# AaltoML/SLAM-module

Measured on AMD Instinct MI355X. Metric: frames/sec ORB extract+match (720p), higher is better.
Workload: dtype u8; 1 GPU; C2+C3: ORB extract 1280x720, 8 levels x1.2, 2000 kpts/frame, FAST thr 20, batch 256 synthetic frames/GPU, + Hamming brute-force best2 + ratio 0.75 of each frame vs the previous (256 pairs, <=2000x2000); batch_per_gpu=256, corner_density=7-9 % of pixels (tools/synth.py defaults)

## Files before the change

include/mi355slam.h:

```cpp
#ifndef MI355SLAM_H
#define MI355SLAM_H

#include <stddef.h>
#include <stdint.h>

#ifdef __cplusplus
extern "C" {
#endif

#define MS_MAX_LEVELS 16
#define MS_ORB_PATCH_RADIUS 19
#define MS_HAMMING_THR_LOW 50
#define MS_HAMMING_THR_HIGH 100
#define MS_HAMMING_MAX 256

typedef enum {
    MS_OK = 0,
    MS_ERR_INVALID = -1,
    MS_ERR_NO_DEVICE = -2,
    MS_ERR_HIP = -3,
    MS_ERR_CAPACITY = -4,
    MS_ERR_NUMERIC = -5,
    MS_ERR_TOO_LATE = -6
} ms_status;
// ... 45 lines not shown
typedef struct {
    int32_t capacity;
    int32_t *count;
    float *x, *y;
    float *angle;
    int32_t *octave;
    uint32_t *desc;
    int32_t *track_id;
} ms_keypoints;

int ms_orb_create(ms_ctx *ctx, const ms_orb_config *cfg, ms_orb **out);
void ms_orb_destroy(ms_orb *orb);

int ms_orb_set_valid_mask(ms_orb *orb, const uint8_t *mask_host);

int ms_orb_extract(ms_orb *orb, const uint8_t *images, int images_on_device, int n_frames,
                   size_t frame_stride, size_t row_stride,
                   const float *track_xy, const int32_t *track_id, const int32_t *n_tracks);

int ms_orb_device_view(ms_orb *orb, ms_keypoints *view);
int ms_orb_download(ms_orb *orb, int frame, float *x, float *y, float *angle, int32_t *octave,
                    uint32_t *desc, int32_t *track_id, int32_t *n);
int ms_orb_capacity(const ms_orb *orb);

#define MS_KEYPOINT_RECORD_BYTES 76
int ms_keypoints_pack(ms_ctx *ctx, const ms_keypoints *view, int frame, int n, const double *bearing, uint8_t *records_host);
int ms_keypoints_unpack(const uint8_t *records, int n, float *x, float *y, float *angle, int32_t *octave, double *bearing, uint32_t *desc);

int ms_orb_set_describe_strip(ms_orb *orb, int r);

int ms_orb_set_resize_plan(ms_orb *orb, int px, int map);

int ms_orb_set_describe_order(ms_orb *orb, int mode);

#define MS_ORB_STAGES 6
int ms_orb_set_profiling(ms_orb *orb, int enable);
int ms_orb_stage_ms(ms_orb *orb, float *ms );
int ms_orb_stage_ms_back(ms_orb *orb, int calls_back, float *ms );
int ms_orb_level_size(const ms_orb *orb, int level, int32_t *w, int32_t *h);
int ms_orb_download_level(ms_orb *orb, int frame, int level, int blurred, uint8_t *dst_host);
int ms_orb_download_detections(ms_orb *orb, int frame, int level, int32_t *x, int32_t *y, int32_t *score, int32_t *n);
int ms_orb_last_candidate_counts(ms_orb *orb, int32_t *out );

int ms_hamming_set_path(ms_ctx *ctx, int path);

int ms_hamming_best2(ms_ctx *ctx, const uint32_t *q, int nq, const uint32_t *t, int nt, int n_pairs,
                     const int32_t *q_bucket, const int32_t *t_bucket, const uint8_t *t_valid,
                     int32_t *best_idx, uint16_t *best_dist, uint16_t *second_dist);

int ms_hamming_best2_sets(ms_ctx *ctx, const uint32_t *q_pool, int q_stride, const int32_t *q_count,
                          const uint32_t *t_pool, int t_stride, const int32_t *t_count,
                          const int32_t *pair_q, const int32_t *pair_t, int n_pairs,
                          int32_t *best_idx, uint16_t *best_dist, uint16_t *second_dist);

int ms_ratio_test(ms_ctx *ctx, const int32_t *best_idx, const uint16_t *best_dist, const uint16_t *second_dist,
                  int n, float lowe_ratio, int max_dist, int32_t *match);

int ms_hamming_candidates(ms_ctx *ctx, const uint32_t *q_desc, int nq, const uint32_t *t_desc,
                          const int32_t *cand_start, const int32_t *cand_idx, const uint8_t *t_skip, const int32_t *t_octave,
                          int32_t *best_idx, uint16_t *best_dist, uint16_t *second_dist, int32_t *best_octave, int32_t *second_octave,
                          int32_t *second_idx );

#define MS_MEDOID_MAX_OBS 256
int ms_descriptor_medoid(ms_ctx *ctx, const uint32_t *desc_pool, const int32_t *obs_start, const int32_t *obs_idx, int n_points,
                         int max_obs, int32_t *best_local, int32_t *best_pool);

// ... 608 lines not shown
```

slam-module_amd/csrc/orb.hip:

```cpp
#include "ms_internal.h"
#include "fast_tiles.h"
#include "describe_order.h"
#include "describe_strips.h"
#include "describe_lanes.h"
#include "describe_steer.h"
#include "describe_brief_index.h"
#include "resize_vpass.h"
#include "resize_plan.h"
#include "orb_geom.h"
#include <cfloat>
#include <cmath>
#include <cstring>

namespace {

using describe_lanes::kHalfPatch;

__device__ __forceinline__ int tile_level(const TileMap &tm, int levels, int t) {
    int l = 0;
#pragma unroll
    for (int k = 1; k < MS_MAX_LEVELS; ++k) l += t >= tm.base[k] ? 1 : 0;
    return l;
}

// ... 358 lines not shown
        for (int r = 0; r < kBlurRows + 6; ++r) {
            const uint8_t *row = img + (uint64_t)reflect101(y0 - 3 + r, h) * pitch;
            uint32_t d = reinterpret_cast<const U32u *>(row + xa)->v;
            if (wave_l) {
                const uint32_t f0 = reinterpret_cast<const U32u *>(row)->v, f1 = reinterpret_cast<const U32u *>(row + 4)->v;
                d = is_l ? __builtin_amdgcn_perm(f1, f0, 0x01020304u) : d;
            }
            if (wave_r) {
                const uint32_t e0 = reinterpret_cast<const U32u *>(row + (w - 8))->v, e1 = reinterpret_cast<const U32u *>(row + (w - 4))->v;
                d = is_r ? __builtin_amdgcn_perm(e1, e0, sel_r) : d;
            }
            e[r] = d & 0x00FF00FFu;
            o[r] = (d >> 8) & 0x00FF00FFu;
        }
    }
    uint8_t *dst = src.slab + (uint64_t)f * TL.slab_stride + G.blur_off;
#pragma unroll
    for (int j = 0; j < kBlurRows; ++j) {
        const uint32_t Ce = vsum7(e + j), Co = vsum7(o + j);
        const uint32_t Le = wave_from_prev(Ce), Lo = wave_from_prev(Co);
        const uint32_t Re = wave_from_next(Ce), Ro = wave_from_next(Co);
        uint32_t o0 = dot2(Lo, 18, 48, 32768u); o0 = dot2(Le, 0, 34, o0); o0 = dot2(Ce, 56, 34, o0); o0 = dot2(Co, 48, 18, o0);
        uint32_t o1 = dot2(Le, 0, 18, 32768u); o1 = dot2(Lo, 0, 34, o1); o1 = dot2(Ce, 48, 48, o1); o1 = dot2(Co, 56, 34, o1); o1 = dot2(Re, 18, 0, o1);
        uint32_t o2 = dot2(Lo, 0, 18, 32768u); o2 = dot2(Ce, 34, 56, o2); o2 = dot2(Co, 48, 48, o2); o2 = dot2(Re, 34, 0, o2); o2 = dot2(Ro, 18, 0, o2);
        uint32_t o3 = dot2(Ce, 18, 48, 32768u); o3 = dot2(Co, 34, 56, o3); o3 = dot2(Re, 48, 18, o3); o3 = dot2(Ro, 34, 0, o3);
        const int y = y0 + j;
        if (y < h && lane >= 1 && lane <= 62 && x < w)
            *reinterpret_cast<uint32_t *>(dst + (uint64_t)y * G.pitch + x) = (o0 >> 16) | ((o1 >> 16) << 8) | ((o2 >> 16) << 16) | ((o3 >> 16) << 24);
    }
}

constexpr int kFastWaves = 8, kFastThreads = 64 * kFastWaves;
constexpr int kFastSeg = 248, kFastRows = 4 * kFastWaves - 2, kFastPosRows = kFastRows + 2, kFastRowsPerWave = 4;
constexpr int kFastPruneMinBlocks = 2 * 4 * 256;
constexpr int kFastPositions = kFastPosRows * (kFastSeg + 2);

__device__ __forceinline__ uint32_t pk_sub(uint32_t a, uint32_t b) {
    return __builtin_bit_cast(uint32_t, (us2_t)(__builtin_bit_cast(us2_t, a) - __builtin_bit_cast(us2_t, b)));
}

__device__ __forceinline__ int mbcnt64(unsigned long long m) {
    return (int)__builtin_amdgcn_mbcnt_hi((uint32_t)(m >> 32), __builtin_amdgcn_mbcnt_lo((uint32_t)m, 0u));
}

__device__ __forceinline__ uint32_t pk_min(uint32_t a, uint32_t b) { return __builtin_bit_cast(uint32_t, __builtin_elementwise_min(__builtin_bit_cast(s2_t, a), __builtin_bit_cast(s2_t, b))); }
__device__ __forceinline__ uint32_t pk_max(uint32_t a, uint32_t b) { return __builtin_bit_cast(uint32_t, __builtin_elementwise_max(__builtin_bit_cast(s2_t, a), __builtin_bit_cast(s2_t, b))); }
__device__ __forceinline__ uint32_t compass_pass(uint32_t n, uint32_t s_, uint32_t e, uint32_t w, uint32_t c, uint32_t T2) {
    const uint32_t a = pk_max(n, s_), b = pk_min(n, s_), cx = pk_max(e, w), d = pk_min(e, w);
    return pk_sub(T2, pk_max(pk_sub(pk_min(a, cx), c), pk_sub(c, pk_max(b, d))));
}

__device__ __forceinline__ int arc_score(const s2_t P[8]) {
    s2_t pmn[8], smn[8];
    pmn[0] = P[0];
    smn[7] = P[7];
#pragma unroll
    for (int k = 1; k < 8; ++k) {
        pmn[k] = __builtin_elementwise_min(pmn[k - 1], P[k]);
        smn[7 - k] = __builtin_elementwise_min(smn[8 - k], P[7 - k]);
    }
    s2_t best = __builtin_elementwise_min(smn[0], pmn[0].yx);
#pragma unroll
    for (int k = 1; k < 8; ++k) best = __builtin_elementwise_max(best, __builtin_elementwise_min(smn[k], pmn[k].yx));
    return max((int)best.x, (int)best.y);
}

__device__ __forceinline__ s2_t pk_mad(uint32_t s, uint32_t r, uint32_t k) {
// ... 657 lines not shown
}

}

struct ms_orb {
    ms_ctx *ctx = nullptr;
    ms_orb_config cfg{};
    PyrGeom geom{};
    TileMap blur_tiles{};
    TileLevels tile_levels{};
    uint8_t *d_block = nullptr;
#define ORB_X_MEMBER(T, name, n) T *d_##name = nullptr;
#define ORB_XL_MEMBER(T, name, n) T *d_##name[MS_MAX_LEVELS] = {nullptr};
    ORB_BLOCK_CONSTANTS(ORB_X_MEMBER, ORB_XL_MEMBER)
    ORB_BLOCK_WORK(ORB_X_MEMBER)
#undef ORB_X_MEMBER
#undef ORB_XL_MEMBER
    size_t cand_count_bytes = 0, score_hist_bytes = 0;
    uint8_t *d_mask = nullptr;
    bool wide[MS_MAX_LEVELS] = {false};
    int resize_px = 0, resize_map = 0;
    int describe_order = describe_order::kDefaultMode;
    int describe_strip = 0;
    bool profiling = false;
    bool blur_valid = false;
    static constexpr int kProfRing = 128;
    hipEvent_t evr[kProfRing][MS_ORB_STAGES + 1] = {{nullptr}};
    hipEvent_t *ev = evr[0];
    long long prof_calls = 0;
    hipStream_t copy_stream = nullptr;
    hipEvent_t ev_copied[4] = {nullptr}, ev_free[4] = {nullptr}, ev_end = nullptr;
    int chunked_frames = 0;
    bool end_recorded = false;
    FrameSrc last_src{};
    int last_frames = 0;
    bool lvl0_in_slab = false;
    uint64_t lvl0_off = 0;
    int lvl0_pitch = 0;
};

#define MS_TRY(x) do { int rc__ = (x); if (rc__ != MS_OK) return rc__; } while (0)

__global__ __launch_bounds__(256) void k_pack_keypoints(const float *__restrict__ x, const float *__restrict__ y, const float *__restrict__ angle,
                                                       const int32_t *__restrict__ octave, const uint32_t *__restrict__ desc, const double *__restrict__ bearing,
                                                       uint64_t base, int n, uint32_t *__restrict__ out) {
    const int i = blockIdx.x * 256 + threadIdx.x;
    if (i >= n * 19) return;
    const int k = i / 19, w = i - 19 * k;
    const uint64_t s = base + (uint64_t)k;
    uint32_t v;
    if (w == 0) v = __float_as_uint(x[s]);
    else if (w == 1) v = __float_as_uint(y[s]);
    else if (w == 2) v = __float_as_uint(angle[s]);
    else if (w < 5) v = (uint32_t)octave[s];
    else if (w < 11) v = bearing ? reinterpret_cast<const uint32_t *>(bearing)[6 * (uint64_t)k + (w - 5)] : 0u;
    else v = desc[s * 8 + (w - 11)];
    out[i] = v;
}

static int orb_take_block(ms_orb *o, const OrbGeom &R, const OrbTables &C) {
    ms_ctx *c = o->ctx;
    const OrbBlock K = orb_block_layout(o->cfg, R, C);
    MS_HIP(c, hipMalloc(reinterpret_cast<void **>(&o->d_block), K.end));
#define ORB_X_BIND(T, name, n) o->d_##name = K.name.at(o->d_block);
#define ORB_XL_BIND(T, name, n) for (int l = 0; l < MS_MAX_LEVELS; ++l) o->d_##name[l] = K.name[l].count ? K.name[l].at(o->d_block) : nullptr;
    ORB_BLOCK_CONSTANTS(ORB_X_BIND, ORB_XL_BIND)
    ORB_BLOCK_WORK(ORB_X_BIND)
#undef ORB_X_BIND
#undef ORB_XL_BIND
    o->cand_count_bytes = K.cand_count.bytes(); o->score_hist_bytes = K.score_hist.bytes();
    std::vector<uint8_t> stage;
    orb_stage_constants(K, R, C, stage);
    MS_HIP(c, hipMemcpyAsync(o->d_block, stage.data(), K.const_end, hipMemcpyHostToDevice, c->stream));
    MS_HIP(c, hipMemsetAsync(o->d_block + K.const_end, 0, K.end - K.const_end, c->stream));
    MS_HIP(c, hipStreamSynchronize(c->stream));
    return MS_OK;
}

static int orb_create_streams(ms_orb *o) {
    ms_ctx *c = o->ctx;
    MS_HIP(c, hipEventCreateWithFlags(&o->ev_end, hipEventDisableTiming));
    if (o->cfg.max_batch < 32) return MS_OK;
    MS_HIP(c, hipStreamCreateWithFlags(&o->copy_stream, hipStreamNonBlocking));
    for (int i = 0; i < 4; ++i) {
        MS_HIP(c, hipEventCreateWithFlags(&o->ev_copied[i], hipEventDisableTiming));
        MS_HIP(c, hipEventCreateWithFlags(&o->ev_free[i], hipEventDisableTiming));
    }
    return MS_OK;
}

extern "C" {

int ms_orb_create(ms_ctx *ctx, const ms_orb_config *cfg, ms_orb **out) {
    if (!ctx || !cfg || !out) return MS_ERR_INVALID;
    *out = nullptr;
    OrbGeom R;
    char why[256];
    const int bad = orb_geometry(*cfg, R, why, sizeof(why));
    if (bad != MS_OK) return ms_fail(ctx, bad, "ms_orb_create: %s", why);
    OrbTables C;
    orb_tables(R.geom, C);
    MS_HIP(ctx, hipSetDevice(ctx->device));
    ms_orb *o = new ms_orb();
    o->ctx = ctx;
    o->cfg = *cfg;
    o->geom = R.geom; o->tile_levels = R.tile_levels; o->blur_tiles = R.blur_tiles;
    o->lvl0_off = R.lvl0_off; o->lvl0_pitch = R.lvl0_pitch;
    for (int l = 1; l < cfg->levels; ++l) o->wide[l] = C.level[l].wide;
    if (orb_take_block(o, R, C) != MS_OK) { ms_orb_destroy(o); return ms_fail(ctx, MS_ERR_HIP, "ms_orb_create: device allocation failed"); }
    if (orb_create_streams(o) != MS_OK) { ms_orb_destroy(o); return ms_fail(ctx, MS_ERR_HIP, "ms_orb_create: stream / event creation failed"); }
    *out = o;
    return MS_OK;
}

void ms_orb_destroy(ms_orb *o) {
    if (!o) return;
    (void)hipSetDevice(o->ctx->device);
    (void)hipStreamSynchronize(o->ctx->stream);
    if (o->d_block) (void)hipFree(o->d_block);
    if (o->d_mask) (void)hipFree(o->d_mask);
    for (auto &set : o->evr) for (int i = 0; i <= MS_ORB_STAGES; ++i) if (set[i]) (void)hipEventDestroy(set[i]);
    if (o->copy_stream) { (void)hipStreamSynchronize(o->copy_stream); (void)hipStreamDestroy(o->copy_stream); }
    for (int i = 0; i < 4; ++i) { if (o->ev_copied[i]) (void)hipEventDestroy(o->ev_copied[i]); if (o->ev_free[i]) (void)hipEventDestroy(o->ev_free[i]); }
    if (o->ev_end) (void)hipEventDestroy(o->ev_end);
    delete o;
}

int ms_orb_capacity(const ms_orb *o) { return o ? o->geom.capacity : MS_ERR_INVALID; }

int ms_orb_set_describe_strip(ms_orb *o, int r) {
    if (!o || r < 0 || r > describe_strips::kMaxStrip) return MS_ERR_INVALID;
    o->describe_strip = r;
    return MS_OK;
}

int ms_orb_set_resize_plan(ms_orb *o, int px, int map) {
    if (!o || (px != 0 && px != 4 && px != 8) || map < resize_plan::kMapAuto || map > resize_plan::kMapByFrame) return MS_ERR_INVALID;
    o->resize_px = px; o->resize_map = map;
    return MS_OK;
}

int ms_orb_set_describe_order(ms_orb *o, int mode) {
    if (!o || mode < 0 || (mode & ~describe_order::kModeMask)) return MS_ERR_INVALID;
    o->describe_order = mode;
    return MS_OK;
}

int ms_orb_set_profiling(ms_orb *o, int enable) {
    if (!o) return MS_ERR_INVALID;
    ms_ctx *c = o->ctx;
    if (enable && !o->evr[0][0])
        for (auto &set : o->evr) for (int i = 0; i <= MS_ORB_STAGES; ++i) MS_HIP(c, hipEventCreate(&set[i]));
    o->profiling = enable != 0;
    return MS_OK;
}

int ms_orb_stage_ms_back(ms_orb *o, int calls_back, float *ms) {
    if (!o || !ms || calls_back < 0 || calls_back >= ms_orb::kProfRing) return MS_ERR_INVALID;
    ms_ctx *c = o->ctx;
    if (!o->evr[0][0] || calls_back >= o->prof_calls) return ms_fail(c, MS_ERR_INVALID, "ms_orb_stage_ms_back: no profiled call %d calls back", calls_back);
    hipEvent_t *set = o->evr[(o->prof_calls - 1 - calls_back) % ms_orb::kProfRing];
    MS_HIP(c, hipEventSynchronize(set[MS_ORB_STAGES]));
    for (int i = 0; i < MS_ORB_STAGES; ++i) MS_HIP(c, hipEventElapsedTime(&ms[i], set[i], set[i + 1]));
    return MS_OK;
}

int ms_orb_stage_ms(ms_orb *o, float *ms) {
    if (!o || !ms) return MS_ERR_INVALID;
    ms_ctx *c = o->ctx;
    if (!o->profiling || o->last_frames == 0) return ms_fail(c, MS_ERR_INVALID, "ms_orb_stage_ms: profiling is off or nothing ran");
    MS_HIP(c, hipEventSynchronize(o->ev[MS_ORB_STAGES]));
    for (int i = 0; i < MS_ORB_STAGES; ++i) MS_HIP(c, hipEventElapsedTime(&ms[i], o->ev[i], o->ev[i + 1]));
    return MS_OK;
}

int ms_orb_set_valid_mask(ms_orb *o, const uint8_t *mask) {
    if (!o) return MS_ERR_INVALID;
    ms_ctx *c = o->ctx;
    MS_HIP(c, hipStreamSynchronize(c->stream));
    if (!mask) { if (o->d_mask) { MS_HIP(c, hipFree(o->d_mask)); o->d_mask = nullptr; } return MS_OK; }
    const size_t n = (size_t)o->cfg.width * o->cfg.height;
    if (!o->d_mask) MS_HIP(c, hipMalloc(reinterpret_cast<void **>(&o->d_mask), n));
    MS_HIP(c, hipMemcpy(o->d_mask, mask, n, hipMemcpyHostToDevice));
    return MS_OK;
}

static int orb_extract_enqueue(ms_orb *o, const uint8_t *images, int on_device, int n_frames, size_t frame_stride, size_t row_stride,
                               const float *track_xy, const int32_t *track_id, const int32_t *n_tracks, bool &counters_dirty);

int ms_orb_extract(ms_orb *o, const uint8_t *images, int on_device, int n_frames, size_t frame_stride, size_t row_stride,
                   const float *track_xy, const int32_t *track_id, const int32_t *n_tracks) {
    if (!o || !images) return MS_ERR_INVALID;
    bool counters_dirty = false;
    const int rc = orb_extract_enqueue(o, images, on_device, n_frames, frame_stride, row_stride, track_xy, track_id, n_tracks, counters_dirty);
    if (rc != MS_OK && counters_dirty) {
        (void)hipMemsetAsync(o->d_cand_count, 0, o->cand_count_bytes, o->ctx->stream);
        (void)hipMemsetAsync(o->d_score_hist, 0, o->score_hist_bytes, o->ctx->stream);
    }
    return rc;
}

static int orb_enqueue_kernels(ms_orb *o, FrameSrc src, int f0, int nf, bool have_tracks, bool have_ids, bool &counters_dirty) {
    ms_ctx *c = o->ctx;
    const PyrGeom &G = o->geom;
    hipStream_t st = c->stream;
    const size_t F = (size_t)f0, T = (size_t)o->cfg.max_tracks, L = (size_t)G.levels;
    src.lvl0 += F * src.lvl0_frame_stride; src.slab += F * G.slab_stride;
    uint32_t *cand = o->d_cand + F * G.cand_stride;
    int32_t *cand_count = o->d_cand_count + F * L, *det_count = o->d_det_count + F * L, *trk_count = o->d_trk_count + F, *last_count = o->d_last_count + F * L;
    const bool prune = (long long)nf * G.ftiles_total > kFastPruneMinBlocks;
    uint32_t *score_hist = prune ? o->d_score_hist + F * L * 256 : nullptr;
    int16_t *det_x = o->d_det_x + F * G.det_stride, *det_y = o->d_det_y + F * G.det_stride;
    uint8_t *det_score = o->d_det_score + F * G.det_stride;
    int stage = 0;
    if (o->profiling) { o->ev = o->evr[o->prof_calls % ms_orb::kProfRing]; ++o->prof_calls; }
#define MS_STAGE_MARK() do { if (o->profiling) MS_HIP(c, hipEventRecord(o->ev[stage++], st)); } while (0)
    MS_STAGE_MARK();
    MsRange pyramid_range("pyramid");
    for (int l = 1; l < G.levels; ++l) {
        dim3 grid(ms_div_up(G.L[l].w, 256), ms_div_up(G.L[l].h, 4 * kResizeRows), nf);
        const ResizeTab RT{o->d_xtab[l], o->d_ytab[l]};
        ResizeArgs RA{};
        if (l == 1) { RA.src = src.lvl0; RA.src_frame_stride = src.lvl0_frame_stride; RA.src_pitch = src.lvl0_pitch; }
        else { RA.src = src.slab + G.L[l - 1].img_off; RA.src_frame_stride = G.slab_stride; RA.src_pitch = G.L[l - 1].pitch; }
        RA.sw = G.L[l - 1].w; RA.sh = G.L[l - 1].h;
        RA.dst = src.slab + G.L[l].img_off; RA.dst_frame_stride = G.slab_stride; RA.dst_pitch = G.L[l].pitch; RA.dw = G.L[l].w; RA.dh = G.L[l].h;
        const resize_plan::Launch P = resize_plan::launch(RA.dw, RA.dh, nf, o->resize_map);
        if (o->d_xtab8[l] && (o->resize_px == 8 || (o->resize_px == 0 && resize_plan::fills_device(P))))
            hipLaunchKernelGGL(k_resize8, dim3(P.grid_x, P.grid_y, P.grid_z), dim3(256), 0, st, RA, Resize8Tab{o->d_xtab8[l], o->d_ytab[l]}, P);
        else if (o->wide[l]) hipLaunchKernelGGL(k_resize<true>, grid, dim3(256), 0, st, RA, RT);
        else hipLaunchKernelGGL(k_resize<false>, grid, dim3(256), 0, st, RA, RT);
        MS_KERNEL_CHECK(c, "k_resize");
    }
    pyramid_range.end();
    MS_STAGE_MARK();
    o->blur_valid = false;
    MS_STAGE_MARK();
    MsRange detect_range("detect");
    counters_dirty = true;
    if (prune) hipLaunchKernelGGL(k_fast<true>, dim3(nf, G.ftiles_total), dim3(kFastThreads), 0, st, src, cand, cand_count, score_hist, o->d_ftile_tab, o->tile_levels);
    else hipLaunchKernelGGL(k_fast<false>, dim3(G.ftiles_total, nf), dim3(kFastThreads), 0, st, src, cand, cand_count, score_hist, o->d_ftile_tab, o->tile_levels);
    MS_KERNEL_CHECK(c, "k_fast");
    MS_STAGE_MARK();
    const bool few = nf * G.levels <= 64;
    if (o->cfg.min_distance > 0.f) {
        if (few) hipLaunchKernelGGL((k_select<true, 1024>), dim3(G.levels, nf), dim3(1024), 0, st, o->d_geom, cand, cand_count, o->d_mask, det_x, det_y, det_score, det_count, score_hist, last_count);
        else hipLaunchKernelGGL((k_select<true, 256>), dim3(G.levels, nf), dim3(256), 0, st, o->d_geom, cand, cand_count, o->d_mask, det_x, det_y, det_score, det_count, score_hist, last_count);
    } else {
        if (few) hipLaunchKernelGGL((k_select<false, 1024>), dim3(G.levels, nf), dim3(1024), 0, st, o->d_geom, cand, cand_count, o->d_mask, det_x, det_y, det_score, det_count, score_hist, last_count);
        else hipLaunchKernelGGL((k_select<false, 256>), dim3(G.levels, nf), dim3(256), 0, st, o->d_geom, cand, cand_count, o->d_mask, det_x, det_y, det_score, det_count, score_hist, last_count);
    }
    MS_KERNEL_CHECK(c, "k_select");
    counters_dirty = false;
    MS_STAGE_MARK();
    if (o->cfg.max_tracks > 0) {
        hipLaunchKernelGGL(k_tracks, dim3(nf), dim3(64), 0, st, o->d_geom, have_tracks ? o->d_track_xy + F * T * 2 : nullptr,
                           (have_tracks && have_ids) ? o->d_track_id + F * T : nullptr, have_tracks ? o->d_n_tracks + F : nullptr, o->d_mask,
                           o->d_trk_x + F * T, o->d_trk_y + F * T, o->d_trk_px + F * T, o->d_trk_py + F * T, o->d_trk_id + F * T, trk_count);
        MS_KERNEL_CHECK(c, "k_tracks");
    }
    MS_STAGE_MARK();
    detect_range.end();
    MsRange describe_range("describe");
    const size_t C = (size_t)G.capacity;
    if (o->describe_order & describe_order::kSpatial)
        hipLaunchKernelGGL(k_slots<true>, dim3(G.levels, nf), dim3(256), 0, st, det_x, det_y, det_count, trk_count, o->d_slot_tab + F * C, o->d_count + F, o->tile_levels, G.det_stride, G.capacity);
    else
        hipLaunchKernelGGL(k_slots<false>, dim3(G.levels, nf), dim3(256), 0, st, det_x, det_y, det_count, trk_count, o->d_slot_tab + F * C, o->d_count + F, o->tile_levels, G.det_stride, G.capacity);
    MS_KERNEL_CHECK(c, "k_slots");
    describe_strips::Plan plan;
    if (!describe_strips::build(nf, G.capacity, 8ll * std::max(c->n_cu, 1), o->describe_strip, plan)) return ms_fail(c, MS_ERR_CAPACITY, "k_describe: %d frames of %d slots exceed the grid", nf, G.capacity);
    hipLaunchKernelGGL(k_describe, dim3(plan.blocks), dim3(256), 0, st, src, o->tile_levels, plan, o->d_moment_tab, o->d_pattern_f,
                       o->d_slot_tab + F * C, G.capacity, G.max_tracks, G.lk_level, o->describe_order & describe_order::kRemap, o->d_trk_x + F * T, o->d_trk_y + F * T, o->d_trk_px + F * T, o->d_trk_py + F * T, o->d_trk_id + F * T, trk_count, o->d_x + F * C, o->d_y + F * C,
                       o->d_angle + F * C, o->d_octave + F * C, o->d_desc + F * C * 8, o->d_track + F * C, o->d_count + F);
    MS_KERNEL_CHECK(c, "k_describe");
    MS_STAGE_MARK();
#undef MS_STAGE_MARK
    return MS_OK;
}

static int orb_extract_enqueue(ms_orb *o, const uint8_t *images, int on_device, int n_frames, size_t frame_stride, size_t row_stride,
                               const float *track_xy, const int32_t *track_id, const int32_t *n_tracks, bool &counters_dirty) {
    ms_ctx *c = o->ctx;
    const PyrGeom &G = o->geom;
    if (n_frames < 1 || n_frames > o->cfg.max_batch) return ms_fail(c, MS_ERR_CAPACITY, "ms_orb_extract: n_frames %d outside [1,%d]", n_frames, o->cfg.max_batch);
    if (row_stride < (size_t)G.width || frame_stride < row_stride * (size_t)(G.height - 1) + G.width)
        return ms_fail(c, MS_ERR_INVALID, "ms_orb_extract: strides smaller than the frame");
    MS_HIP(c, hipSetDevice(c->device));
    hipStream_t st = c->stream;
    MS_TRY(ms_ctx_order_after_downloads(c));
    FrameSrc src{};
    src.slab = o->d_slab;
    const bool have_tracks = track_xy && n_tracks && o->cfg.max_tracks > 0;
    if (have_tracks) {
        const size_t T = o->cfg.max_tracks;
        MS_HIP(c, hipMemcpyAsync(o->d_track_xy, track_xy, (size_t)n_frames * T * 2 * sizeof(float), hipMemcpyHostToDevice, st));
        MS_HIP(c, hipMemcpyAsync(o->d_n_tracks, n_tracks, (size_t)n_frames * sizeof(int32_t), hipMemcpyHostToDevice, st));
        if (track_id) MS_HIP(c, hipMemcpyAsync(o->d_track_id, track_id, (size_t)n_frames * T * sizeof(int32_t), hipMemcpyHostToDevice, st));
    }
    const bool aligned = on_device && (reinterpret_cast<uintptr_t>(images) % 16 == 0) && (row_stride % 16 == 0) && (frame_stride % 16 == 0);
    if (aligned) {
        src.lvl0 = images; src.lvl0_frame_stride = frame_stride; src.lvl0_pitch = (int)row_stride;
        o->lvl0_in_slab = false;
        MS_TRY(orb_enqueue_kernels(o, src, 0, n_frames, have_tracks, track_id != nullptr, counters_dirty));
    } else {
        uint8_t *dst = o->d_slab + o->lvl0_off;
        src.lvl0 = dst; src.lvl0_frame_stride = G.slab_stride; src.lvl0_pitch = o->lvl0_pitch;
        o->lvl0_in_slab = true;
        const bool whole = row_stride == (size_t)o->lvl0_pitch;
        const size_t frame_bytes = row_stride * (size_t)(G.height - 1) + G.width;
        auto copy_frames = [&](int f0, int nf, hipStream_t cs) -> int {
            if (whole && nf > 1) {
                MS_HIP(c, hipMemcpy2DAsync(dst + (size_t)f0 * G.slab_stride, G.slab_stride, images + (size_t)f0 * frame_stride, frame_stride, frame_bytes, nf, hipMemcpyHostToDevice, cs));
            } else {
                for (int f = f0; f < f0 + nf; ++f) {
                    if (whole) MS_HIP(c, hipMemcpyAsync(dst + (size_t)f * G.slab_stride, images + (size_t)f * frame_stride, frame_bytes, hipMemcpyHostToDevice, cs));
                    else MS_HIP(c, hipMemcpy2DAsync(dst + (size_t)f * G.slab_stride, o->lvl0_pitch, images + (size_t)f * frame_stride, row_stride, G.width, G.height, hipMemcpyHostToDevice, cs));
                }
            }
            return MS_OK;
        };
        const int kChunks = 4;
        const bool chunked = !on_device && !o->profiling && n_frames >= 8 * kChunks && o->copy_stream != nullptr;
        if (on_device) {
            dim3 grid(ms_div_up(G.width, 256), G.height, n_frames);
            hipLaunchKernelGGL(k_copy_level0, grid, dim3(256), 0, st, images, (uint64_t)frame_stride, (uint64_t)row_stride, o->d_slab,
                               G.slab_stride, o->lvl0_off, G.width, G.height, o->lvl0_pitch);
            MS_KERNEL_CHECK(c, "k_copy_level0");
            MS_TRY(orb_enqueue_kernels(o, src, 0, n_frames, have_tracks, track_id != nullptr, counters_dirty));
        } else if (!chunked) {
            MS_TRY(copy_frames(0, n_frames, st));
            MS_TRY(orb_enqueue_kernels(o, src, 0, n_frames, have_tracks, track_id != nullptr, counters_dirty));
        } else {
            const int per = ms_div_up(n_frames, kChunks);
            const bool same_split = o->chunked_frames == n_frames;
            if (!same_split && o->end_recorded) MS_HIP(c, hipStreamWaitEvent(o->copy_stream, o->ev_end, 0));
            for (int k = 0; k < kChunks; ++k) {
                const int f0 = k * per, nf = std::min(per, n_frames - f0);
                if (nf <= 0) break;
                if (same_split) MS_HIP(c, hipStreamWaitEvent(o->copy_stream, o->ev_free[k], 0));
                MS_TRY(copy_frames(f0, nf, o->copy_stream));
                MS_HIP(c, hipEventRecord(o->ev_copied[k], o->copy_stream));
                MS_HIP(c, hipStreamWaitEvent(st, o->ev_copied[k], 0));
                MS_TRY(orb_enqueue_kernels(o, src, f0, nf, have_tracks, track_id != nullptr, counters_dirty));
                MS_HIP(c, hipEventRecord(o->ev_free[k], st));
            }
            o->chunked_frames = n_frames;
        }
        if (!chunked) o->chunked_frames = 0;
    }
    if (aligned) o->chunked_frames = 0;
    if (o->ev_end) { MS_HIP(c, hipEventRecord(o->ev_end, st)); o->end_recorded = true; }
    o->last_src = src;
    o->last_frames = n_frames;
    return MS_OK;
}

int ms_keypoints_pack(ms_ctx *c, const ms_keypoints *view, int frame, int n, const double *bearing, uint8_t *records_host) {
    if (!c || !view || !view->x || !view->y || !view->angle || !view->octave || !view->desc || frame < 0 || n < 0 || n > view->capacity || (n && !records_host))
        return MS_ERR_INVALID;
    if (n == 0) return MS_OK;
    MS_HIP(c, hipSetDevice(c->device));
    void *scratch = nullptr;
    MS_TRY(ms_scratch(c, (size_t)n * MS_KEYPOINT_RECORD_BYTES, &scratch));
    hipLaunchKernelGGL(k_pack_keypoints, dim3(ms_div_up(n * 19, 256)), dim3(256), 0, c->stream, view->x, view->y, view->angle, view->octave, view->desc, bearing,
                       (uint64_t)frame * (uint64_t)view->capacity, n, static_cast<uint32_t *>(scratch));
    MS_KERNEL_CHECK(c, "k_pack_keypoints");
    MS_HIP(c, hipMemcpyAsync(records_host, scratch, (size_t)n * MS_KEYPOINT_RECORD_BYTES, hipMemcpyDeviceToHost, c->stream));
    MS_HIP(c, hipStreamSynchronize(c->stream));
    return MS_OK;
}

int ms_keypoints_unpack(const uint8_t *records, int n, float *x, float *y, float *angle, int32_t *octave, double *bearing, uint32_t *desc) {
    if (n < 0 || (n && !records)) return MS_ERR_INVALID;
    for (int k = 0; k < n; ++k) {
        const uint8_t *r = records + (size_t)k * MS_KEYPOINT_RECORD_BYTES;
        int32_t o1, o2;
// ... 13 lines not shown
    if (!o || !v) return MS_ERR_INVALID;
    v->capacity = o->geom.capacity; v->count = o->d_count; v->x = o->d_x; v->y = o->d_y; v->angle = o->d_angle;
    v->octave = o->d_octave; v->desc = o->d_desc; v->track_id = o->d_track;
    return MS_OK;
}

int ms_orb_download(ms_orb *o, int frame, float *x, float *y, float *angle, int32_t *octave, uint32_t *desc, int32_t *track_id, int32_t *n) {
    if (!o || !n) return MS_ERR_INVALID;
    ms_ctx *c = o->ctx;
    if (frame < 0 || frame >= o->last_frames) return ms_fail(c, MS_ERR_INVALID, "ms_orb_download: frame %d not in last batch", frame);
    MS_HIP(c, hipStreamSynchronize(c->stream));
    int32_t cnt = 0;
    MS_HIP(c, hipMemcpy(&cnt, o->d_count + frame, sizeof(int32_t), hipMemcpyDeviceToHost));
    const size_t cap = o->geom.capacity, b = (size_t)frame * cap, k = (size_t)cnt;
    if (x) MS_HIP(c, hipMemcpy(x, o->d_x + b, k * 4, hipMemcpyDeviceToHost));
    if (y) MS_HIP(c, hipMemcpy(y, o->d_y + b, k * 4, hipMemcpyDeviceToHost));
    if (angle) MS_HIP(c, hipMemcpy(angle, o->d_angle + b, k * 4, hipMemcpyDeviceToHost));
    if (octave) MS_HIP(c, hipMemcpy(octave, o->d_octave + b, k * 4, hipMemcpyDeviceToHost));
    if (desc) MS_HIP(c, hipMemcpy(desc, o->d_desc + b * 8, k * 32, hipMemcpyDeviceToHost));
    if (track_id) MS_HIP(c, hipMemcpy(track_id, o->d_track + b, k * 4, hipMemcpyDeviceToHost));
    *n = cnt;
    return MS_OK;
}

int ms_orb_last_candidate_counts(ms_orb *o, int32_t *out) {
    if (!o || !out) return MS_ERR_INVALID;
    ms_ctx *c = o->ctx;
    if (o->last_frames < 1) return ms_fail(c, MS_ERR_INVALID, "ms_orb_last_candidate_counts: nothing ran");
    MS_HIP(c, hipStreamSynchronize(c->stream));
    MS_HIP(c, hipMemcpy(out, o->d_last_count, sizeof(int32_t) * (size_t)o->last_frames * o->geom.levels, hipMemcpyDeviceToHost));
    return MS_OK;
}

int ms_orb_level_size(const ms_orb *o, int level, int32_t *w, int32_t *h) {
    if (!o || level < 0 || level >= o->geom.levels || !w || !h) return MS_ERR_INVALID;
    *w = o->geom.L[level].w; *h = o->geom.L[level].h;
    return MS_OK;
}

int ms_orb_download_level(ms_orb *o, int frame, int level, int blurred, uint8_t *dst) {
    if (!o || !dst) return MS_ERR_INVALID;
    ms_ctx *c = o->ctx;
    if (frame < 0 || frame >= o->last_frames || level < 0 || level >= o->geom.levels) return ms_fail(c, MS_ERR_INVALID, "ms_orb_download_level: bad frame/level");
    MS_HIP(c, hipStreamSynchronize(c->stream));
    const LevelGeom &L = o->geom.L[level];
    const uint8_t *p; size_t pitch;
    if (blurred) {
        if (!o->blur_valid) {
            hipLaunchKernelGGL(k_blur, dim3(o->geom.btiles_total, o->last_frames), dim3(256), 0, c->stream, o->last_src, o->tile_levels, o->blur_tiles);
            MS_KERNEL_CHECK(c, "k_blur");
            MS_HIP(c, hipStreamSynchronize(c->stream));
            o->blur_valid = true;
        }
        p = o->d_slab + (size_t)frame * o->geom.slab_stride + L.blur_off; pitch = L.pitch;
    }
    else if (level == 0) { p = o->last_src.lvl0 + (size_t)frame * o->last_src.lvl0_frame_stride; pitch = o->last_src.lvl0_pitch; }
    else { p = o->d_slab + (size_t)frame * o->geom.slab_stride + L.img_off; pitch = L.pitch; }
    MS_HIP(c, hipMemcpy2D(dst, L.w, p, pitch, L.w, L.h, hipMemcpyDeviceToHost));
    return MS_OK;
}

int ms_orb_download_detections(ms_orb *o, int frame, int level, int32_t *x, int32_t *y, int32_t *score, int32_t *n) {
    if (!o || !n) return MS_ERR_INVALID;
    ms_ctx *c = o->ctx;
    if (frame < 0 || frame >= o->last_frames || level < 0 || level >= o->geom.levels) return ms_fail(c, MS_ERR_INVALID, "ms_orb_download_detections: bad frame/level");
    MS_HIP(c, hipStreamSynchronize(c->stream));
// ... 16 lines not shown
```

slam-module_amd/csrc/orb_geom.h:

```cpp
#pragma once
#include <algorithm>
#include <cmath>
#include <cstdint>
#include <vector>
#include "ms_check.h"
#include "ms_geometry.h"
#include "ms_layout.h"
#include "fast_tiles.h"
#include "describe_order.h"
#include "describe_lanes.h"
#include "resize_plan.h"

#if defined(__HIPCC__)
typedef uint2 orb_u2; typedef uint4 orb_u4; typedef float4 orb_f4;
#else
struct alignas(8) orb_u2 { uint32_t x, y; };
struct alignas(16) orb_u4 { uint32_t x, y, z, w; };
struct alignas(16) orb_f4 { float x, y, z, w; };
#endif

namespace {

constexpr int kPatchRadius = MS_ORB_PATCH_RADIUS;
constexpr int kMaxQuota = 4096;
constexpr int kResizeRows = 5;
constexpr int kBlurSeg = 248;
constexpr int kBlurRows = 18;

struct LevelGeom {
    int32_t w, h, pitch, quota;
    int32_t min_dist;
    int32_t det_base;
    int32_t cand_cap;
    int32_t btiles_x, btile_base;
    uint32_t btiles_inv;
    uint64_t img_off, blur_off;
    uint64_t cand_off;
    float scale;
};

struct PyrGeom {
    int32_t levels, lk_level, fast_threshold, max_kpts, max_tracks, capacity;
    int32_t det_stride;
    int32_t width, height, btiles_total, ftiles_total;
    uint64_t slab_stride, cand_stride;
    int32_t umax[16];
    LevelGeom L[MS_MAX_LEVELS];
};

struct TileMap { int32_t base[MS_MAX_LEVELS + 1]; };

struct TileLevel { int32_t w, h, pitch, btiles_x, cand_cap; uint32_t btiles_inv; uint64_t img_off, blur_off, cand_off; float scale; int32_t det_base;
                   int32_t sel_k; };
struct TileLevels { TileLevel L[MS_MAX_LEVELS]; uint64_t slab_stride, cand_stride; int32_t levels, fast_threshold; };

struct OrbGeom {
    PyrGeom geom;
    TileLevels tile_levels;
    TileMap blur_tiles;
    std::vector<uint32_t> ftile_tab;
    uint64_t lvl0_off;
    int32_t lvl0_pitch;
};

#define ORB_GEOM_FAIL(code, ...) return ms_why(code, why, why_bytes, __VA_ARGS__)

inline int orb_geometry(const ms_orb_config &cfg, OrbGeom &R, char *why, size_t why_bytes) {
    if (cfg.levels < 1 || cfg.levels > MS_MAX_LEVELS || cfg.max_kpts < 1 || cfg.max_batch < 1 || cfg.max_tracks < 0 ||
        cfg.lk_track_level < 0 || cfg.lk_track_level >= cfg.levels || cfg.fast_threshold < 1 || cfg.fast_threshold > 254 ||
        !(cfg.scale_factor > 1.0f) || !(cfg.min_distance >= 0.f) || cfg.width > 32767 || cfg.height > 32767 ||
        (int64_t)cfg.width * cfg.height >= (1 << 24))
        ORB_GEOM_FAIL(MS_ERR_INVALID, "unsupported configuration");
    R = OrbGeom{};
    PyrGeom &G = R.geom;
    G.levels = cfg.levels; G.lk_level = cfg.lk_track_level; G.fast_threshold = cfg.fast_threshold;
    G.max_kpts = cfg.max_kpts; G.max_tracks = cfg.max_tracks;
    G.width = cfg.width; G.height = cfg.height;
    int32_t w[MS_MAX_LEVELS], h[MS_MAX_LEVELS], quota[MS_MAX_LEVELS];
    float sf[MS_MAX_LEVELS];
    msgeo::level_sizes(cfg.levels, cfg.scale_factor, cfg.width, cfg.height, w, h);
    msgeo::level_quotas(cfg.levels, cfg.scale_factor, cfg.max_kpts, quota);
    msgeo::scale_factors(cfg.levels, cfg.scale_factor, sf);
    msgeo::umax(G.umax);
    uint64_t off = 0, coff = 0;
    int det_base = 0, bt = 0;
    for (int l = 0; l < cfg.levels; ++l) {
        if (w[l] < 2 * kPatchRadius + 2 || h[l] < 2 * kPatchRadius + 2 || quota[l] > kMaxQuota)
            ORB_GEOM_FAIL(MS_ERR_INVALID, "level %d is %dx%d (min 40x40) / quota %d (max %d)", l, w[l], h[l], quota[l], kMaxQuota);
        if ((int64_t)ms_div_up(w[l], kBlurSeg) * ms_div_up(h[l], 4 * kBlurRows) >= 65536)
            ORB_GEOM_FAIL(MS_ERR_CAPACITY, "level %d (%dx%d) needs more than 65535 blur tiles", l, w[l], h[l]);
        LevelGeom &L = G.L[l];
        L.w = w[l]; L.h = h[l]; L.pitch = (int)ms_align_up(w[l], 64); L.quota = quota[l]; L.scale = sf[l];
        {
            const double su = std::min(w[l], h[l]) / 720.0 * 0.8;
            L.min_dist = (int)std::floor(cfg.min_distance * su + 0.5);
        }
        L.det_base = det_base; det_base += quota[l];
        L.img_off = off; off += (uint64_t)L.pitch * L.h;
        L.blur_off = off; off += (uint64_t)L.pitch * L.h;
        L.cand_cap = (int32_t)ms_align_up((size_t)(((w[l] + 1) / 2) * ((h[l] + 1) / 2) + 256), 4);
        L.cand_off = coff; coff += L.cand_cap;
        L.btiles_x = ms_div_up(w[l], kBlurSeg); L.btile_base = bt; bt += L.btiles_x * ms_div_up(h[l], 4 * kBlurRows);
        L.btiles_inv = (uint32_t)(((1ull << 32) + L.btiles_x - 1) / L.btiles_x);
    }
    G.btiles_total = bt;
    {
        std::vector<fast_tiles::Tile> cover;
        for (int l = 0; l < cfg.levels; ++l) {
            cover.clear();
            fast_tiles::cover(w[l], h[l], cover);
            for (const fast_tiles::Tile &t : cover) {
                R.ftile_tab.push_back((uint32_t)l | ((uint32_t)t.S << 4));
                R.ftile_tab.push_back((uint32_t)t.X0 | ((uint32_t)t.Y0 << 16));
            }
            if (!cover.empty() && (cover.back().X0 > 0xFFFF || cover.back().Y0 > 0xFFFF))
                ORB_GEOM_FAIL(MS_ERR_CAPACITY, "level %d (%dx%d) is beyond the detector's tile table (65535 px)", l, w[l], h[l]);
        }
    }
    const size_t ftiles = R.ftile_tab.size() / 2;
    G.ftiles_total = (int)ftiles;
    if (ftiles > 65535) ORB_GEOM_FAIL(MS_ERR_CAPACITY, "%zu detector tiles per frame (max 65535)", ftiles);
    G.det_stride = std::max(cfg.max_kpts, det_base);
    G.capacity = G.det_stride + cfg.max_tracks;
    if (G.capacity >= (1 << (32 - describe_order::kSlotShift)))
        ORB_GEOM_FAIL(MS_ERR_CAPACITY, "%d output slots per frame (max %d)", G.capacity, (1 << (32 - describe_order::kSlotShift)) - 1);
    for (int l = 0; l < cfg.levels; ++l) {
        const LevelGeom &L = G.L[l];
        const int sel_k = (cfg.min_distance > 0.f && L.min_dist >= 2) ? std::min(4 * L.quota, kMaxQuota) : L.quota;
        R.tile_levels.L[l] = TileLevel{L.w, L.h, L.pitch, L.btiles_x, L.cand_cap, L.btiles_inv, L.img_off, L.blur_off, L.cand_off, L.scale, L.det_base, sel_k};
    }
    for (int l = 0; l <= MS_MAX_LEVELS; ++l) R.blur_tiles.base[l] = l < cfg.levels ? G.L[l].btile_base : bt;
    G.slab_stride = ms_align_up(off, 256); G.cand_stride = coff;
    R.tile_levels.slab_stride = G.slab_stride; R.tile_levels.cand_stride = G.cand_stride; R.tile_levels.levels = G.levels; R.tile_levels.fast_threshold = G.fast_threshold;
    R.lvl0_off = G.L[0].img_off; R.lvl0_pitch = G.L[0].pitch;
    return MS_OK;
}
#undef ORB_GEOM_FAIL

struct OrbResizeTables { std::vector<int16_t> xt, yt; std::vector<uint32_t> x8; bool wide = false; };

inline void orb_resize_tables(const PyrGeom &G, int l, OrbResizeTables &T) {
    const int sw = G.L[l - 1].w, sh = G.L[l - 1].h, dw = G.L[l].w, dh = G.L[l].h;
    std::vector<int16_t> xo, xc, yo, yc;
    msgeo::resize_tables(sw, dw, true, xo, xc);
    msgeo::resize_tables(sh, dh, false, yo, yc);
    const int wpad = ms_div_up(dw, 4) * 4, hpad = ms_div_up(dh, kResizeRows) * kResizeRows;
    std::vector<int16_t> xt(4 * (size_t)wpad), yt(4 * (size_t)hpad);
    for (int d = 0; d < dw; ++d) { xt[4 * d] = xo[d]; xt[4 * d + 1] = xc[2 * d]; xt[4 * d + 2] = xc[2 * d + 1]; xt[4 * d + 3] = 0; }
    for (int d = 0; d < dh; ++d) {
        yt[4 * d] = (int16_t)std::min(std::max((int)yo[d], 0), sh - 1);
        yt[4 * d + 1] = (int16_t)std::min(std::max((int)yo[d] + 1, 0), sh - 1);
        yt[4 * d + 2] = yc[2 * d]; yt[4 * d + 3] = yc[2 * d + 1];
    }
    for (int d = dw; d < wpad; ++d) for (int k = 0; k < 4; ++k) xt[4 * d + k] = xt[4 * (dw - 1) + k];
    for (int d = dh; d < hpad; ++d) for (int k = 0; k < 4; ++k) yt[4 * d + k] = yt[4 * (dh - 1) + k];
    T.wide = false;
    for (int d = 0; d + 3 < dw; d += 4) if (xo[d + 3] + 1 - xo[d] > 7) T.wide = true;
    T.x8.clear();
    if (T.wide || !resize_plan::rows_shared(yt.data(), dh, sh) || !resize_plan::build_columns(xo.data(), xc.data(), sw, dw, T.x8)) T.x8.clear();
    T.xt.swap(xt); T.yt.swap(yt);
}

inline void orb_describe_tables(const int32_t *umax, std::vector<uint32_t> &mt, std::vector<float> &pf) {
    static const int8_t pattern[1024] = {
#include "orb_pattern.inc"
    };
    mt.assign(64 * 4 + 32 * 4 + 64 + 64 * 2, 0u);
    for (int lane = 0; lane < 64; ++lane)
        for (int t = 0; t < 4; ++t) mt[lane * 4 + t] = describe_lanes::disc_mask(lane, t, umax);
    uint32_t taps[64 * 4];
// ... 99 lines not shown
```

slam-module_amd/mi355slam/__init__.py:

```python
import ctypes as C
import os
import weakref

import numpy as np

_HERE = os.path.dirname(os.path.abspath(__file__))
LIB_PATH = os.path.join(os.path.dirname(_HERE), "lib", "libmi355slam.so")
MAX_LEVELS = 16

u8p = C.POINTER(C.c_uint8)
i32p = C.POINTER(C.c_int32)
u32p = C.POINTER(C.c_uint32)
u16p = C.POINTER(C.c_uint16)
f32p = C.POINTER(C.c_float)
f64p = C.POINTER(C.c_double)


class MsError(RuntimeError):
    pass


class OrbConfig(C.Structure):
    _fields_ = [("width", C.c_int32), ("height", C.c_int32), ("levels", C.c_int32), ("scale_factor", C.c_float),
                ("max_kpts", C.c_int32), ("lk_track_level", C.c_int32), ("fast_threshold", C.c_int32),
# ... 254 lines not shown
    def device_view(self):
        v = KeypointsView()
        self.ctx.check(lib().ms_orb_device_view(self._h, C.byref(v)), "ms_orb_device_view")
        return v

    def download(self, frame):
        cap = self.capacity
        out = dict(x=np.zeros(cap, np.float32), y=np.zeros(cap, np.float32), angle=np.zeros(cap, np.float32),
                   octave=np.zeros(cap, np.int32), desc=np.zeros((cap, 8), np.uint32), track_id=np.zeros(cap, np.int32))
        n = C.c_int32()
        self.ctx.check(lib().ms_orb_download(self._h, frame, _vp(out["x"]), _vp(out["y"]), _vp(out["angle"]), _vp(out["octave"]),
                                             _vp(out["desc"]), _vp(out["track_id"]), C.byref(n)), "ms_orb_download")
        return {k: v[:n.value].copy() for k, v in out.items()}

    def pack_keypoints(self, frame, bearing=None):
        self.ctx.sync()
        v = self.device_view()
        cnt = np.zeros(1, np.int32)
        self.ctx.check(lib().ms_dev_download(self.ctx._h, _vp(cnt), C.c_void_p(v.count + 4 * frame), C.c_size_t(4)), "ms_dev_download")
        n = int(cnt[0])
        out = np.zeros((n, 76), np.uint8)
        db = None if bearing is None else self.ctx.upload(np.ascontiguousarray(bearing, np.float64).reshape(n, 3))
        self.ctx.check(lib().ms_keypoints_pack(self.ctx._h, C.byref(v), frame, n, _vp(db), _vp(out)), "ms_keypoints_pack")
        return out

    def set_describe_strip(self, r):
        self.ctx.check(lib().ms_orb_set_describe_strip(self._h, int(r)), "ms_orb_set_describe_strip")

    def set_resize_plan(self, px=0, map=0):
        self.ctx.check(lib().ms_orb_set_resize_plan(self._h, int(px), int(map)), "ms_orb_set_resize_plan")

    def set_describe_order(self, mode):
        self.ctx.check(lib().ms_orb_set_describe_order(self._h, int(mode)), "ms_orb_set_describe_order")

    def set_profiling(self, enable=True):
        self.ctx.check(lib().ms_orb_set_profiling(self._h, int(enable)), "ms_orb_set_profiling")

    def stage_ms(self):
        ms = (C.c_float * 6)()
        self.ctx.check(lib().ms_orb_stage_ms(self._h, ms), "ms_orb_stage_ms")
        return dict(zip(("resize", "blur", "fast", "select", "tracks", "describe"), [float(v) for v in ms]))

    def stage_ms_back(self, calls_back):
        ms = (C.c_float * 6)()
        self.ctx.check(lib().ms_orb_stage_ms_back(self._h, int(calls_back), ms), "ms_orb_stage_ms_back")
        return dict(zip(("resize", "blur", "fast", "select", "tracks", "describe"), [float(v) for v in ms]))

    def level_size(self, level):
        w, h = C.c_int32(), C.c_int32()
        self.ctx.check(lib().ms_orb_level_size(self._h, level, C.byref(w), C.byref(h)), "ms_orb_level_size")
        return w.value, h.value

    def download_level(self, frame, level, blurred=False):
        w, h = self.level_size(level)
        out = np.zeros((h, w), np.uint8)
        self.ctx.check(lib().ms_orb_download_level(self._h, frame, level, int(blurred), _vp(out)), "ms_orb_download_level")
        return out

    def download_detections(self, frame, level):
        q = self.capacity
        x, y, s = np.zeros(q, np.int32), np.zeros(q, np.int32), np.zeros(q, np.int32)
        n = C.c_int32()
        self.ctx.check(lib().ms_orb_download_detections(self._h, frame, level, _vp(x), _vp(y), _vp(s), C.byref(n)), "ms_orb_download_detections")
        return x[:n.value].copy(), y[:n.value].copy(), s[:n.value].copy()

    def last_candidate_counts(self):
# ... 1887 lines not shown
```

Before: 181,400 frames/s.

## Run level-0 FAST detection on a side stream overlapping pyramid resize

```diff
diff --git a/include/mi355slam.h b/include/mi355slam.h
--- a/include/mi355slam.h
+++ b/include/mi355slam.h
@@ -101,6 +101,9 @@
 int ms_orb_set_resize_plan(ms_orb *orb, int px, int map);
 
 int ms_orb_set_describe_order(ms_orb *orb, int mode);
+
+int ms_orb_set_fast_overlap(ms_orb *orb, int mode);
+int ms_orb_last_fast_launches(const ms_orb *orb, int32_t *launches, int32_t *pruning);
 
 #define MS_ORB_STAGES 6
 int ms_orb_set_profiling(ms_orb *orb, int enable);
diff --git a/slam-module_amd/csrc/orb.hip b/slam-module_amd/csrc/orb.hip
--- a/slam-module_amd/csrc/orb.hip
+++ b/slam-module_amd/csrc/orb.hip
@@ -414,7 +414,6 @@
 
 constexpr int kFastWaves = 8, kFastThreads = 64 * kFastWaves;
 constexpr int kFastSeg = 248, kFastRows = 4 * kFastWaves - 2, kFastPosRows = kFastRows + 2, kFastRowsPerWave = 4;
-constexpr int kFastPruneMinBlocks = 2 * 4 * 256;
 constexpr int kFastPositions = kFastPosRows * (kFastSeg + 2);
 
 __device__ __forceinline__ uint32_t pk_sub(uint32_t a, uint32_t b) {
@@ -1138,6 +1137,12 @@
     hipEvent_t ev_copied[4] = {nullptr}, ev_free[4] = {nullptr}, ev_end = nullptr;
     int chunked_frames = 0;
     bool end_recorded = false;
+    int ftiles_level0 = 0;
+    int fast_overlap = 0;
+    int fast_launches = 0, fast_pruning = 0;
+    hipStream_t side_stream = nullptr;
+    bool side_owned = false;
+    hipEvent_t ev_fork = nullptr, ev_join = nullptr;
     FrameSrc last_src{};
     int last_frames = 0;
     bool lvl0_in_slab = false;
@@ -1183,15 +1188,28 @@
     return MS_OK;
 }
 
+static int orb_create_side_stream(ms_orb *o) {
+    ms_ctx *c = o->ctx;
+    if (o->side_stream) return MS_OK;
+    if (!o->ev_fork) MS_HIP(c, hipEventCreateWithFlags(&o->ev_fork, hipEventDisableTiming));
+    if (!o->ev_join) MS_HIP(c, hipEventCreateWithFlags(&o->ev_join, hipEventDisableTiming));
+    if (o->copy_stream) { o->side_stream = o->copy_stream; return MS_OK; }
+    MS_HIP(c, hipStreamCreateWithFlags(&o->side_stream, hipStreamNonBlocking));
+    o->side_owned = true;
+    return MS_OK;
+}
+
 static int orb_create_streams(ms_orb *o) {
     ms_ctx *c = o->ctx;
     MS_HIP(c, hipEventCreateWithFlags(&o->ev_end, hipEventDisableTiming));
-    if (o->cfg.max_batch < 32) return MS_OK;
-    MS_HIP(c, hipStreamCreateWithFlags(&o->copy_stream, hipStreamNonBlocking));
-    for (int i = 0; i < 4; ++i) {
-        MS_HIP(c, hipEventCreateWithFlags(&o->ev_copied[i], hipEventDisableTiming));
-        MS_HIP(c, hipEventCreateWithFlags(&o->ev_free[i], hipEventDisableTiming));
-    }
+    if (o->cfg.max_batch >= 32) {
+        MS_HIP(c, hipStreamCreateWithFlags(&o->copy_stream, hipStreamNonBlocking));
+        for (int i = 0; i < 4; ++i) {
+            MS_HIP(c, hipEventCreateWithFlags(&o->ev_copied[i], hipEventDisableTiming));
+            MS_HIP(c, hipEventCreateWithFlags(&o->ev_free[i], hipEventDisableTiming));
+        }
+    }
+    if (orb_fast_split_auto(o->cfg.max_batch, o->ftiles_level0, o->geom.ftiles_total)) MS_TRY(orb_create_side_stream(o));
     return MS_OK;
 }
 
@@ -1211,7 +1229,7 @@
     o->ctx = ctx;
     o->cfg = *cfg;
     o->geom = R.geom; o->tile_levels = R.tile_levels; o->blur_tiles = R.blur_tiles;
-    o->lvl0_off = R.lvl0_off; o->lvl0_pitch = R.lvl0_pitch;
+    o->lvl0_off = R.lvl0_off; o->lvl0_pitch = R.lvl0_pitch; o->ftiles_level0 = R.ftiles_level0;
     for (int l = 1; l < cfg->levels; ++l) o->wide[l] = C.level[l].wide;
     if (orb_take_block(o, R, C) != MS_OK) { ms_orb_destroy(o); return ms_fail(ctx, MS_ERR_HIP, "ms_orb_create: device allocation failed"); }
     if (orb_create_streams(o) != MS_OK) { ms_orb_destroy(o); return ms_fail(ctx, MS_ERR_HIP, "ms_orb_create: stream / event creation failed"); }
@@ -1229,6 +1247,9 @@
     if (o->copy_stream) { (void)hipStreamSynchronize(o->copy_stream); (void)hipStreamDestroy(o->copy_stream); }
     for (int i = 0; i < 4; ++i) { if (o->ev_copied[i]) (void)hipEventDestroy(o->ev_copied[i]); if (o->ev_free[i]) (void)hipEventDestroy(o->ev_free[i]); }
     if (o->ev_end) (void)hipEventDestroy(o->ev_end);
+    if (o->side_owned) { (void)hipStreamSynchronize(o->side_stream); (void)hipStreamDestroy(o->side_stream); }
+    if (o->ev_fork) (void)hipEventDestroy(o->ev_fork);
+    if (o->ev_join) (void)hipEventDestroy(o->ev_join);
     delete o;
 }
 
@@ -1249,6 +1270,16 @@
 int ms_orb_set_describe_order(ms_orb *o, int mode) {
     if (!o || mode < 0 || (mode & ~describe_order::kModeMask)) return MS_ERR_INVALID;
     o->describe_order = mode;
+    return MS_OK;
+}
+
+int ms_orb_set_fast_overlap(ms_orb *o, int mode) {
+    if (!o || mode < 0 || mode > 2) return MS_ERR_INVALID;
+    if (mode == 2 && o->geom.levels > 1) {
+        MS_HIP(o->ctx, hipSetDevice(o->ctx->device));
+        MS_TRY(orb_create_side_stream(o));
+    }
+    o->fast_overlap = mode;
     return MS_OK;
 }
 
@@ -1300,13 +1331,17 @@
     bool counters_dirty = false;
     const int rc = orb_extract_enqueue(o, images, on_device, n_frames, frame_stride, row_stride, track_xy, track_id, n_tracks, counters_dirty);
     if (rc != MS_OK && counters_dirty) {
+        if (o->side_stream) {
+            (void)hipEventRecord(o->ev_join, o->side_stream);
+            (void)hipStreamWaitEvent(o->ctx->stream, o->ev_join, 0);
+        }
         (void)hipMemsetAsync(o->d_cand_count, 0, o->cand_count_bytes, o->ctx->stream);
         (void)hipMemsetAsync(o->d_score_hist, 0, o->score_hist_bytes, o->ctx->stream);
     }
     return rc;
 }
 
-static int orb_enqueue_kernels(ms_orb *o, FrameSrc src, int f0, int nf, bool have_tracks, bool have_ids, bool &counters_dirty) {
+static int orb_enqueue_kernels(ms_orb *o, FrameSrc src, int f0, int nf, bool have_tracks, bool have_ids, bool in_pieces, bool &counters_dirty) {
     ms_ctx *c = o->ctx;
     const PyrGeom &G = o->geom;
     hipStream_t st = c->stream;
@@ -1316,12 +1351,28 @@
     int32_t *cand_count = o->d_cand_count + F * L, *det_count = o->d_det_count + F * L, *trk_count = o->d_trk_count + F, *last_count = o->d_last_count + F * L;
     const bool prune = (long long)nf * G.ftiles_total > kFastPruneMinBlocks;
     uint32_t *score_hist = prune ? o->d_score_hist + F * L * 256 : nullptr;
+    const int tiles0 = o->ftiles_level0, tiles1 = G.ftiles_total - tiles0;
+    const bool split = o->side_stream && tiles1 > 0 && o->fast_overlap != 1 &&
+                       (o->fast_overlap == 2 || (!in_pieces && orb_fast_split_auto(nf, tiles0, G.ftiles_total)));
+    auto launch_fast = [&](hipStream_t s, int tile0, int tiles) {
+        ++o->fast_launches; o->fast_pruning += prune;
+        if (prune) hipLaunchKernelGGL(k_fast<true>, dim3(nf, tiles), dim3(kFastThreads), 0, s, src, cand, cand_count, score_hist, o->d_ftile_tab + tile0, o->tile_levels);
+        else hipLaunchKernelGGL(k_fast<false>, dim3(tiles, nf), dim3(kFastThreads), 0, s, src, cand, cand_count, score_hist, o->d_ftile_tab + tile0, o->tile_levels);
+    };
     int16_t *det_x = o->d_det_x + F * G.det_stride, *det_y = o->d_det_y + F * G.det_stride;
     uint8_t *det_score = o->d_det_score + F * G.det_stride;
     int stage = 0;
     if (o->profiling) { o->ev = o->evr[o->prof_calls % ms_orb::kProfRing]; ++o->prof_calls; }
 #define MS_STAGE_MARK() do { if (o->profiling) MS_HIP(c, hipEventRecord(o->ev[stage++], st)); } while (0)
     MS_STAGE_MARK();
+    if (split) {
+        MS_HIP(c, hipEventRecord(o->ev_fork, st));
+        MS_HIP(c, hipStreamWaitEvent(o->side_stream, o->ev_fork, 0));
+        counters_dirty = true;
+        launch_fast(o->side_stream, 0, tiles0);
+        MS_KERNEL_CHECK(c, "k_fast");
+        MS_HIP(c, hipEventRecord(o->ev_join, o->side_stream));
+    }
     MsRange pyramid_range("pyramid");
     for (int l = 1; l < G.levels; ++l) {
         dim3 grid(ms_div_up(G.L[l].w, 256), ms_div_up(G.L[l].h, 4 * kResizeRows), nf);
@@ -1344,9 +1395,9 @@
     MS_STAGE_MARK();
     MsRange detect_range("detect");
     counters_dirty = true;
-    if (prune) hipLaunchKernelGGL(k_fast<true>, dim3(nf, G.ftiles_total), dim3(kFastThreads), 0, st, src, cand, cand_count, score_hist, o->d_ftile_tab, o->tile_levels);
-    else hipLaunchKernelGGL(k_fast<false>, dim3(G.ftiles_total, nf), dim3(kFastThreads), 0, st, src, cand, cand_count, score_hist, o->d_ftile_tab, o->tile_levels);
+    if (split) launch_fast(st, tiles0, tiles1); else launch_fast(st, 0, G.ftiles_total);
     MS_KERNEL_CHECK(c, "k_fast");
+    if (split) MS_HIP(c, hipStreamWaitEvent(st, o->ev_join, 0));
     MS_STAGE_MARK();
     const bool few = nf * G.levels <= 64;
     if (o->cfg.min_distance > 0.f) {
@@ -1394,6 +1445,7 @@
         return ms_fail(c, MS_ERR_INVALID, "ms_orb_extract: strides smaller than the frame");
     MS_HIP(c, hipSetDevice(c->device));
     hipStream_t st = c->stream;
+    o->fast_launches = o->fast_pruning = 0;
     MS_TRY(ms_ctx_order_after_downloads(c));
     FrameSrc src{};
     src.slab = o->d_slab;
@@ -1408,7 +1460,7 @@
     if (aligned) {
         src.lvl0 = images; src.lvl0_frame_stride = frame_stride; src.lvl0_pitch = (int)row_stride;
         o->lvl0_in_slab = false;
-        MS_TRY(orb_enqueue_kernels(o, src, 0, n_frames, have_tracks, track_id != nullptr, counters_dirty));
+        MS_TRY(orb_enqueue_kernels(o, src, 0, n_frames, have_tracks, track_id != nullptr, false, counters_dirty));
     } else {
         uint8_t *dst = o->d_slab + o->lvl0_off;
         src.lvl0 = dst; src.lvl0_frame_stride = G.slab_stride; src.lvl0_pitch = o->lvl0_pitch;
@@ -1433,10 +1485,10 @@
             hipLaunchKernelGGL(k_copy_level0, grid, dim3(256), 0, st, images, (uint64_t)frame_stride, (uint64_t)row_stride, o->d_slab,
                                G.slab_stride, o->lvl0_off, G.width, G.height, o->lvl0_pitch);
             MS_KERNEL_CHECK(c, "k_copy_level0");
-            MS_TRY(orb_enqueue_kernels(o, src, 0, n_frames, have_tracks, track_id != nullptr, counters_dirty));
+            MS_TRY(orb_enqueue_kernels(o, src, 0, n_frames, have_tracks, track_id != nullptr, false, counters_dirty));
         } else if (!chunked) {
             MS_TRY(copy_frames(0, n_frames, st));
-            MS_TRY(orb_enqueue_kernels(o, src, 0, n_frames, have_tracks, track_id != nullptr, counters_dirty));
+            MS_TRY(orb_enqueue_kernels(o, src, 0, n_frames, have_tracks, track_id != nullptr, false, counters_dirty));
         } else {
             const int per = ms_div_up(n_frames, kChunks);
             const bool same_split = o->chunked_frames == n_frames;
@@ -1448,7 +1500,7 @@
                 MS_TRY(copy_frames(f0, nf, o->copy_stream));
                 MS_HIP(c, hipEventRecord(o->ev_copied[k], o->copy_stream));
                 MS_HIP(c, hipStreamWaitEvent(st, o->ev_copied[k], 0));
-                MS_TRY(orb_enqueue_kernels(o, src, f0, nf, have_tracks, track_id != nullptr, counters_dirty));
+                MS_TRY(orb_enqueue_kernels(o, src, f0, nf, have_tracks, track_id != nullptr, true, counters_dirty));
                 MS_HIP(c, hipEventRecord(o->ev_free[k], st));
             }
             o->chunked_frames = n_frames;
@@ -1528,6 +1580,12 @@
     return MS_OK;
 }
 
+int ms_orb_last_fast_launches(const ms_orb *o, int32_t *launches, int32_t *pruning) {
+    if (!o || !launches || !pruning) return MS_ERR_INVALID;
+    *launches = o->fast_launches; *pruning = o->fast_pruning;
+    return MS_OK;
+}
+
 int ms_orb_level_size(const ms_orb *o, int level, int32_t *w, int32_t *h) {
     if (!o || level < 0 || level >= o->geom.levels || !w || !h) return MS_ERR_INVALID;
     *w = o->geom.L[level].w; *h = o->geom.L[level].h;
diff --git a/slam-module_amd/csrc/orb_geom.h b/slam-module_amd/csrc/orb_geom.h
--- a/slam-module_amd/csrc/orb_geom.h
+++ b/slam-module_amd/csrc/orb_geom.h
@@ -24,6 +24,7 @@
 constexpr int kPatchRadius = MS_ORB_PATCH_RADIUS;
 constexpr int kMaxQuota = 4096;
 constexpr int kResizeRows = 5;
+constexpr int kFastPruneMinBlocks = 2 * 4 * 256;
 constexpr int kBlurSeg = 248;
 constexpr int kBlurRows = 18;
 
@@ -59,6 +60,7 @@
     TileLevels tile_levels;
     TileMap blur_tiles;
     std::vector<uint32_t> ftile_tab;
+    int32_t ftiles_level0;
     uint64_t lvl0_off;
     int32_t lvl0_pitch;
 };
@@ -113,6 +115,7 @@
                 R.ftile_tab.push_back((uint32_t)l | ((uint32_t)t.S << 4));
                 R.ftile_tab.push_back((uint32_t)t.X0 | ((uint32_t)t.Y0 << 16));
             }
+            if (l == 0) R.ftiles_level0 = (int32_t)(R.ftile_tab.size() / 2);
             if (!cover.empty() && (cover.back().X0 > 0xFFFF || cover.back().Y0 > 0xFFFF))
                 ORB_GEOM_FAIL(MS_ERR_CAPACITY, "level %d (%dx%d) is beyond the detector's tile table (65535 px)", l, w[l], h[l]);
         }
@@ -136,6 +139,10 @@
     return MS_OK;
 }
 #undef ORB_GEOM_FAIL
+
+inline bool orb_fast_split_auto(int nf, int ftiles_level0, int ftiles_total) {
+    return (long long)nf * std::min(ftiles_level0, ftiles_total - ftiles_level0) > kFastPruneMinBlocks;
+}
 
 struct OrbResizeTables { std::vector<int16_t> xt, yt; std::vector<uint32_t> x8; bool wide = false; };
 
diff --git a/slam-module_amd/mi355slam/__init__.py b/slam-module_amd/mi355slam/__init__.py
--- a/slam-module_amd/mi355slam/__init__.py
+++ b/slam-module_amd/mi355slam/__init__.py
@@ -310,6 +310,14 @@
 
     def set_describe_order(self, mode):
         self.ctx.check(lib().ms_orb_set_describe_order(self._h, int(mode)), "ms_orb_set_describe_order")
+
+    def set_fast_overlap(self, mode):
+        self.ctx.check(lib().ms_orb_set_fast_overlap(self._h, int(mode)), "ms_orb_set_fast_overlap")
+
+    def last_fast_launches(self):
+        n, p = C.c_int32(), C.c_int32()
+        self.ctx.check(lib().ms_orb_last_fast_launches(self._h, C.byref(n), C.byref(p)), "ms_orb_last_fast_launches")
+        return n.value, p.value
 
     def set_profiling(self, enable=True):
         self.ctx.check(lib().ms_orb_set_profiling(self._h, int(enable)), "ms_orb_set_profiling")
```

Measured after the change: 184,600 frames/s, median of 6. 1.7% higher.
